# SelennLamson/AntsRL

Hardware: AMD Instinct MI355X
Metric: ant-steps/sec (ants x envs x steps/s), 256^2 grid (higher is better)
Workload: dtype f64 ant kinematics / f32 grids

## Files before the change

antsrl_amd/csrc/antsrl_capi.hip:

```cpp
#include <hip/hip_runtime.h>
#include <stdarg.h>
#include <stdio.h>
#include <math.h>
#include <stdlib.h>
#include <string.h>
#include <new>

#include "antsrl_device.h"

hipError_t antsrl_launch_act(const KP &p, const int8_t *rot, const int8_t *ph, int cur, float *obs,
                             float *agent_state, float *reward, uint8_t *done, int flags,
                             const double *jitter, int out_buf, hipStream_t st);
bool antsrl_act_fits(const KP &p);
bool antsrl_act_needs_hbm_maps(const KP &p);
hipError_t antsrl_launch_sweep(const KP &p, int cur, hipStream_t st);
hipError_t antsrl_launch_update(const KP &p, const double *jitter, int out_buf, hipStream_t st, int phases = 15);
hipError_t antsrl_launch_collect_full(const KP &p, hipStream_t st);
hipError_t antsrl_launch_reset(const KP &p, const AntsInit *in, hipStream_t st);
hipError_t antsrl_launch_set_activation(const KP &p, const float *act, hipStream_t st);
hipError_t antsrl_launch_read_state(const KP &p, int which, int cur, void *dst, hipStream_t st);
hipError_t antsrl_launch_perceptive_field(const KP &p, uint8_t *dst, hipStream_t st);
hipError_t antsrl_launch_generate(const KP &p, const AntsGen &g, uint64_t seed, hipStream_t st);
hipError_t antsrl_launch_phero_wall_clear(const KP &p, hipStream_t st, int buf = 0);
hipError_t antsrl_launch_phero_renorm(const KP &p, hipStream_t st);
bool antsrl_meta_supported(const KP &p);
hipError_t antsrl_launch_move(const KP &p, const int8_t *rot, const int8_t *ph, uint8_t *done, int do_step, uint32_t seq,
                              hipStream_t st);
hipError_t antsrl_launch_perceive(const KP &p, int cur, float *obs, float *agent_state, float *reward, int flags,
                                  uint32_t seq, hipStream_t st, const PolArgs *pol, uint32_t obs_pitch);
bool antsrl_inloop_policy_supported(const KP &p);
hipError_t antsrl_launch_policy_pack(unsigned char *pack, const float *w1, const float *b1, const float *w2, const float *b2,
                                     const float *w3, const float *b3, int F, hipStream_t st);
hipError_t antsrl_launch_meta_rebase(const KP &p, hipStream_t st);
bool antsrl_update_move_supported(const KP &p);
hipError_t antsrl_launch_update_move(const KP &p, int out_buf, double g_dep, double inv_g_dep, const int8_t *rot,
                                     const int8_t *ph, uint8_t *done, uint32_t seq, hipStream_t st, bool with_frames);
int antsrl_perceive_run(const KP &p);
hipError_t antsrl_launch_copy16(void *dst, const void *src, size_t bytes, hipStream_t st);

struct AntsHandle {
    AntsCfg cfg;
    KP p;
    int cur;
    int steps_since_update;
    bool need_full_collect;
    bool is_reset;
    bool episode_over;
    size_t ws_bytes;
    AntsGen gen;
    bool has_gen;
    uint64_t episode_seed;
    int host_timestep;
    long long sweeps;
    bool obs_bf16;
    uint32_t obs_pitch;
    bool need_wall_clear;
    hipEvent_t ev[ANTSRL_TIMING_EVENTS];
    bool ev_armed;
    uint32_t obs_seq;
    PolArgs pol;
    bool pend_update;
    KP pend_p;
    int pend_out_buf;
    int phase_next;
};

static thread_local char g_err[512] = "";

static int fail(int code, const char *fmt, ...)
{
    va_list ap;
    va_start(ap, fmt);
    vsnprintf(g_err, sizeof(g_err), fmt, ap);
    va_end(ap);
    return code;
}

static int hip_fail(hipError_t e, const char *what)
{
    return fail(ANTSRL_E_DEVICE, "%s: %s", what, hipGetErrorString(e));
}

extern "C" int antsrl_abi_version(void) { return ANTSRL_ABI_VERSION; }
extern "C" size_t antsrl_cfg_size(void) { return sizeof(AntsCfg); }
extern "C" const char *antsrl_last_error(void) { return g_err; }

static void fill_kp(const AntsCfg *c, KP *p);

static int validate(const AntsCfg *c)
{
    if (!c) return fail(ANTSRL_E_INVALID, "cfg is NULL");
    if (c->abi_version != ANTSRL_ABI_VERSION)
        return fail(ANTSRL_E_INVALID, "AntsCfg.abi_version %d != library %d", c->abi_version, ANTSRL_ABI_VERSION);
    if (c->n_envs < 1 || c->n_ants < 1 || c->w < 1 || c->h < 1)
        return fail(ANTSRL_E_INVALID, "n_envs, n_ants, w, h must be >= 1");
    if ((long long)c->w * c->h > (1ll << 30)) return fail(ANTSRL_E_INVALID, "grid too large");
    if (c->n_envs > 65535)
        return fail(ANTSRL_E_INVALID, "n_envs must be <= 65535 per handle (shard larger batches over handles / GPUs)");
    if (c->n_phero < 1 || c->n_phero > ANTSRL_MAX_PHERO)
        return fail(ANTSRL_E_INVALID, "n_phero must be in 1..%d", ANTSRL_MAX_PHERO);
    if (c->n_rocks < 0 || c->n_rocks > 32) return fail(ANTSRL_E_INVALID, "n_rocks must be in 0..32");
    if (c->perception_radius < 0 || 2 * c->perception_radius + 1 > ANTSRL_MAX_PSIDE)
        return fail(ANTSRL_E_INVALID, "perception side must be <= %d", ANTSRL_MAX_PSIDE);
    if (c->n_channels < 1 || c->n_channels > ANTSRL_MAX_CHANNELS)
        return fail(ANTSRL_E_INVALID, "n_channels must be in 1..%d", ANTSRL_MAX_CHANNELS);
    for (int k = 0; k < c->n_channels; ++k) {
        const int kind = c->channel_kind[k];
        if (kind < ANTSRL_CH_ANTS || kind > ANTSRL_CH_ROCKS) return fail(ANTSRL_E_INVALID, "bad channel kind");
        if (kind == ANTSRL_CH_PHERO && (c->channel_arg[k] < 0 || c->channel_arg[k] >= c->n_phero))
            return fail(ANTSRL_E_INVALID, "pheromone channel index out of range");
        if (kind == ANTSRL_CH_PHERO && !c->has_max_val)
            return fail(ANTSRL_E_INVALID, "a perceived pheromone needs max_val (RL_api.py:125 divides by it)");
        if (kind == ANTSRL_CH_ROCKS && c->n_rocks == 0)
            return fail(ANTSRL_E_INVALID, "rocks perceived but n_rocks == 0");
    }
    if (c->filter_radius < 0 || c->filter_radius > ANTSRL_MAX_FILTER_RADIUS)
        return fail(ANTSRL_E_INVALID, "filter_radius must be in 0..%d", ANTSRL_MAX_FILTER_RADIUS);
    if (c->reward_kind < ANTSRL_REWARD_NONE || c->reward_kind > ANTSRL_REWARD_ALL)
        return fail(ANTSRL_E_INVALID, "bad reward_kind");
    if (c->has_max_val && !(c->phero_max_val > 0)) return fail(ANTSRL_E_INVALID, "phero_max_val must be > 0");
    if (c->act_path < ANTSRL_ACT_AUTO || c->act_path > ANTSRL_ACT_SINGLE_KERNEL) return fail(ANTSRL_E_INVALID, "bad act_path");
    if (c->env_id_base < 0 || (long long)c->env_id_base + c->n_envs > 0x7fffffffll)
        return fail(ANTSRL_E_INVALID, "env_id_base must be >= 0 and env_id_base + n_envs must fit 31 bits");
    if (c->n_envs_total != 0 && (long long)c->n_envs_total < (long long)c->env_id_base + c->n_envs)
        return fail(ANTSRL_E_INVALID, "n_envs_total %d < env_id_base + n_envs = %lld (0 = that sum)", c->n_envs_total,
                    (long long)c->env_id_base + c->n_envs);
    if (c->act_path == ANTSRL_ACT_CELL_META) {
        KP kp;
        fill_kp(c, &kp);
        if (!kp.meta)
            return fail(ANTSRL_E_UNSUPPORTED, "ANTSRL_ACT_CELL_META needs 2 pheromone channels, the generator's channel order "
                                              "([Ants, Phero0, Phero1, Anthill, Walls, Food(, Rocks)]), a perception of 128..368 values "
                                              "per ant over at most 64 cells, and at most 4096 ants per env");
    }
    return ANTSRL_OK;
}

static bool use_scaled(const AntsCfg *c)
{
    return c->phero_mode == ANTSRL_PHERO_AUTO && c->filter_radius == 0 && c->filter[0] > 0.5 &&
           c->filter[0] <= 1.0 && c->phero_threshold >= 0.0;
}

static bool use_interleaved(const AntsCfg *c)
{
    static const bool off = PROF_ENV("ANTSRL_NO_INTERLEAVE") != nullptr;
    return !off && use_scaled(c) && c->n_phero == 2;
}

static size_t carve(const AntsCfg *c, DState *s, unsigned char *base)
{
    const size_t E = c->n_envs, N = c->n_ants, G = (size_t)c->w * c->h, Cn = c->n_phero, R = c->n_rocks;
    const size_t words = (G + 31) / 32;
    size_t off = 0;
    auto take = [&](size_t bytes) -> unsigned char * {
        unsigned char *ptr = base ? base + off : nullptr;
        off = (off + bytes + 255) / 256 * 256;
        return ptr;
    };
// ... 190 lines not shown
{
    if (!h || !init) return fail(ANTSRL_E_INVALID, "NULL handle or init");
    if (!init->ants_xyt || !init->seed || !init->walls || !init->food || !init->anthill_xyr)
        return fail(ANTSRL_E_INVALID, "AntsInit: ants_xyt, seed, walls, food, anthill_xyr are required");
    if (h->p.R > 0 && !init->rocks) return fail(ANTSRL_E_INVALID, "AntsInit.rocks is NULL but n_rocks > 0");
    h->pend_update = false;
    h->phase_next = 0;
    hipError_t e = antsrl_launch_reset(h->p, init, (hipStream_t)stream);
    if (e != hipSuccess) return hip_fail(e, "reset");
    h->p.deposit_strength = h->cfg.deposit_strength;
    h->cur = 0; h->steps_since_update = 0; h->need_full_collect = true; h->is_reset = true; h->episode_over = false;
    h->sweeps = 0; h->need_wall_clear = h->p.scaled && init->phero != nullptr;
    h->host_timestep = 1; h->obs_seq = 0;
    set_decay(h);
    return ANTSRL_OK;
}

static int check_gen_seed(const AntsHandle *h, const AntsGen &g, uint64_t seed)
{
    const uint64_t top = (uint64_t)h->p.env_id_base + (uint64_t)h->p.E;
    const uint64_t lim = 0xFFFFFFFFull / 5u;
    if (g.rng_kind == ANTSRL_RNG_REFERENCE && (top > lim || seed > lim - top))
        return fail(ANTSRL_E_INVALID, "ANTSRL_RNG_REFERENCE: (episode_seed + env_id_base + n_envs) * 5 must stay below 2^32 (np.random.seed)");
    return ANTSRL_OK;
}

static int do_generate(AntsHandle *h, uint64_t seed, hipStream_t st)
{
    int rc = check_gen_seed(h, h->gen, seed);
    if (rc) return rc;
    h->pend_update = false;
    h->phase_next = 0;
    hipError_t e = antsrl_launch_generate(h->p, h->gen, seed, st);
    if (e != hipSuccess) return hip_fail(e, "generate");
    h->p.deposit_strength = h->cfg.deposit_strength;
    h->cur = 0; h->steps_since_update = 0; h->need_full_collect = true; h->is_reset = true; h->episode_over = false;
    h->sweeps = 0; h->need_wall_clear = false; h->host_timestep = 1; h->obs_seq = 0;
    h->episode_seed = seed;
    set_decay(h);
    return ANTSRL_OK;
}

extern "C" int antsrl_generate(AntsHandle *h, const AntsGen *gen, uint64_t episode_seed, void *stream)
{
    if (!h || !gen) return fail(ANTSRL_E_INVALID, "NULL handle or gen");
    if (gen->n_food_discs < 0 || gen->n_food_discs > ANTSRL_MAX_FOOD_DISCS)
        return fail(ANTSRL_E_INVALID, "n_food_discs must be in 0..%d", ANTSRL_MAX_FOOD_DISCS);
    if (gen->food_rmin < 0 || gen->food_rmax < gen->food_rmin) return fail(ANTSRL_E_INVALID, "bad food radii");
    if (gen->wall_kind == ANTSRL_WALLS_BERNOULLI) {
        if (!(gen->wall_density >= 0.0 && gen->wall_density <= 1.0)) return fail(ANTSRL_E_INVALID, "bad wall_density");
    } else if (gen->wall_kind == ANTSRL_WALLS_PERLIN) {
        if (!(gen->wall_density >= -1.0 && gen->wall_density <= 1.0) || gen->perlin_octaves < 1 || gen->perlin_octaves > 8 ||
            !(gen->perlin_scale > 0.0) || !(gen->perlin_persistence > 0.0) || !(gen->perlin_lacunarity > 0.0))
            return fail(ANTSRL_E_INVALID, "bad Perlin wall parameters (density in [-1, 1], 1..8 octaves, positive "
                                          "scale / persistence / lacunarity)");
    } else if (gen->wall_kind == ANTSRL_WALLS_INPUT) {
        if (!gen->walls_input) return fail(ANTSRL_E_INVALID, "ANTSRL_WALLS_INPUT needs AntsGen.walls_input");
    } else {
        return fail(ANTSRL_E_INVALID, "bad wall_kind %d", gen->wall_kind);
    }
    if (gen->rng_kind != ANTSRL_RNG_COUNTER && gen->rng_kind != ANTSRL_RNG_REFERENCE)
        return fail(ANTSRL_E_INVALID, "bad rng_kind %d", gen->rng_kind);
    if (gen->rng_kind == ANTSRL_RNG_REFERENCE) {
        if (gen->wall_kind == ANTSRL_WALLS_BERNOULLI && gen->wall_density != 0.0)
            return fail(ANTSRL_E_UNSUPPORTED, "the reference has no Bernoulli walls generator: with ANTSRL_RNG_REFERENCE use "
                                              "ANTSRL_WALLS_PERLIN, ANTSRL_WALLS_INPUT or wall_density 0");
    }
    int rc = check_gen_seed(h, *gen, episode_seed);
    if (rc) return rc;
    h->gen = *gen;
    h->has_gen = true;
    return do_generate(h, episode_seed, (hipStream_t)stream);
}

static int bf16_unsupported()
{
    return fail(ANTSRL_E_UNSUPPORTED, "bfloat16 observations on the single-kernel path (k_act) need 2 pheromone channels, the "
                                      "generator's channel order ([Ants, Phero0, Phero1, Anthill, Walls, Food(, Rocks)]), a perception of "
                                      "at most 64 cells and a grid whose bit maps fit LDS (up to ~600k cells); the cell-meta path "
                                      "(ANTSRL_Q_CELL_META) has no grid limit");
}

extern "C" int antsrl_set_obs_format(AntsHandle *h, int format)
{
    if (!h) return fail(ANTSRL_E_INVALID, "NULL handle");
    if (format != ANTSRL_OBS_F32 && format != ANTSRL_OBS_BF16) return fail(ANTSRL_E_INVALID, "bad observation format %d", format);
    if ((format == ANTSRL_OBS_BF16) != h->obs_bf16) h->obs_pitch = 0;
    h->obs_bf16 = format == ANTSRL_OBS_BF16;
    if (!h->obs_bf16) h->pol = PolArgs{};
    return ANTSRL_OK;
}

extern "C" int antsrl_set_obs_row_stride(AntsHandle *h, int32_t stride_elems)
{
    if (!h) return fail(ANTSRL_E_INVALID, "NULL handle");
    const int32_t row = h->p.PP * h->p.K, esz = h->obs_bf16 ? 2 : 4;
    if (stride_elems == 0 || stride_elems == row) {
        h->obs_pitch = 0;
        return ANTSRL_OK;
    }
    if (stride_elems < row || ((long long)stride_elems * esz) % 128 != 0 || stride_elems > row + 128 / esz)
        return fail(ANTSRL_E_INVALID, "obs row stride %d: 0 (dense) or the row's %d elements rounded up to whole 128-byte lines (%d)",
                    stride_elems, row, (row * esz + 127) / 128 * 128 / esz);
    if (!h->p.meta) return fail(ANTSRL_E_UNSUPPORTED, "antsrl_set_obs_row_stride needs the cell-meta path (ANTSRL_Q_CELL_META)");
    if (h->pol.pack)
        return fail(ANTSRL_E_UNSUPPORTED, "a padded observation row stride and the in-loop policy exclude each other (the net reads a "
                                          "dense tile image): switch the policy off first (antsrl_set_inloop_policy with w1 == NULL)");
    h->obs_pitch = (uint32_t)stride_elems;
    return ANTSRL_OK;
}

static int hip_fail(hipError_t e, const char *what);
static int flush_pending(AntsHandle *h, hipStream_t st)
{
    if (!h->pend_update) return ANTSRL_OK;
    h->pend_update = false;
    hipError_t e = antsrl_launch_update(h->pend_p, nullptr, h->pend_out_buf, st);
    if (e != hipSuccess) return hip_fail(e, "deferred update");
    return ANTSRL_OK;
}

static int not_reset(const AntsHandle *h)
{
    if (h->episode_over)
        return fail(ANTSRL_E_INVALID, "the episode is over and its auto-reset was refused (episode seed past np.random.seed's 32 bits): "
                                      "call antsrl_reset or antsrl_generate");
    return fail(ANTSRL_E_INVALID, "antsrl_reset has not been called on this handle");
}

static int mid_update(const AntsHandle *h)
{
    return fail(ANTSRL_E_INVALID, "an Environment.update is in progress (antsrl_update_phase %d of 4 is next): finish it first", h->phase_next);
}

static int meta_observe(AntsHandle *h, const int8_t *rot, const int8_t *ph, float *obs, float *agent_state,
                        float *reward, uint8_t *done, bool stepping, hipStream_t st, bool timed)
{
    hipError_t e;
    if (obs && h->obs_pitch != 0 && h->obs_pitch != (uint32_t)(h->p.PP * h->p.K) && h->pol.pack && h->obs_bf16)
        return fail(ANTSRL_E_UNSUPPORTED, "a padded observation row stride and the in-loop policy exclude each other");
    if (h->obs_seq >= META_NEVER - 2) {
        e = antsrl_launch_meta_rebase(h->p, st);
        if (e != hipSuccess) return hip_fail(e, "explored-stamp rebase");
        h->obs_seq = 0;
    }
    h->obs_seq++;
    bool frames = false;
    if (h->pend_update && stepping) {
        h->pend_update = false;
        frames = h->pol.pack != nullptr;
        if (const char *s = PROF_ENV("ANTSRL_FRAMES")) frames = atoi(s) != 0;
        e = antsrl_launch_update_move(h->p, h->pend_out_buf, h->pend_p.g_dep, h->pend_p.inv_g_dep, rot, ph, done, h->obs_seq, st, frames);
        if (e != hipSuccess) return hip_fail(e, "update + move");
    } else {
        int rc = flush_pending(h, st);
        if (rc) return rc;
        e = antsrl_launch_move(h->p, rot, ph, done, stepping ? 1 : 0, h->obs_seq, st);
        if (e != hipSuccess) return hip_fail(e, "move");
    }
    if (timed) (void)hipEventRecord(h->ev[2], st);
    e = antsrl_launch_perceive(h->p, h->cur, obs, agent_state, reward,
                               (stepping ? ACT_STEP : 0) | (obs ? ACT_HAS_OBS : 0) | (frames ? ACT_FRAMES : 0) |
                                   ((obs || h->pol.pack) && h->obs_bf16 ? ACT_OBS_BF16 : 0),
                               h->obs_seq, st, &h->pol, h->obs_pitch);
    if (e == hipErrorNotSupported)
        return fail(ANTSRL_E_UNSUPPORTED, "a padded observation row stride and the in-loop policy exclude each other (the net reads a dense tile image)");
    if (e != hipSuccess) return hip_fail(e, "perceive");
    return ANTSRL_OK;
}

static int do_step(AntsHandle *h, const int8_t *rot, const int8_t *ph, float *obs, float *agent_state,
                   float *reward, uint8_t *done, hipStream_t st, bool fused_update = false,
                   const double *jitter = nullptr, bool timed = false)
{
    if (ph && h->p.C != 2)
        return fail(ANTSRL_E_INVALID, "pheromone actions need exactly 2 pheromone channels (ants.py:89-96)");
    if (h->steps_since_update > 0) h->need_full_collect = true;
    if (h->p.meta) {
        int rc = meta_observe(h, rot, ph, obs, agent_state, reward, done, true, st, timed);
        if (rc) return rc;
        h->steps_since_update++;
        return ANTSRL_OK;
    }
    if (obs && h->obs_pitch) return fail(ANTSRL_E_UNSUPPORTED, "antsrl_set_obs_row_stride needs the cell-meta path (ANTSRL_Q_CELL_META)");
    if (timed) (void)hipEventRecord(h->ev[2], st);
    static const int ablate = PROF_ENV("ANTSRL_ABLATE") ? atoi(PROF_ENV("ANTSRL_ABLATE")) & ~15 : 0;
    hipError_t e = antsrl_launch_act(h->p, rot, ph, h->cur, obs, agent_state, reward, done,
                                     ACT_STEP | (obs ? ACT_HAS_OBS : 0) | (fused_update ? ACT_FUSED_UPDATE : 0) | ablate |
                                         (obs && h->obs_bf16 ? ACT_OBS_BF16 : 0),
                                     jitter, h->p.scaled ? 0 : h->cur ^ 1, st);
    if (e == hipErrorNotSupported) return bf16_unsupported();
    if (e != hipSuccess) return hip_fail(e, "step");
    h->steps_since_update++;
    return ANTSRL_OK;
}

static int do_update(AntsHandle *h, const double *jitter, hipStream_t st, bool sweep_done,
                     bool update_fused = false, bool may_defer = false)
{
    hipError_t e;
    int frc = flush_pending(h, st);
    if (frc) return frc;
    if (h->p.scaled) {
        if (h->p.g_dep < 1e-20) {
            e = antsrl_launch_phero_renorm(h->p, st);
            if (e != hipSuccess) return hip_fail(e, "pheromone renorm");
            h->sweeps = 0;
            set_decay(h);
        }
        if (h->need_wall_clear) {
            e = antsrl_launch_phero_wall_clear(h->p, st);
            if (e != hipSuccess) return hip_fail(e, "pheromone wall clear");
            h->need_wall_clear = false;
        }
    } else if (!sweep_done) {
        e = antsrl_launch_sweep(h->p, h->cur, st);
        if (e != hipSuccess) return hip_fail(e, "pheromone sweep");
    }
    if (!update_fused) {
        if (may_defer && !jitter && !h->need_full_collect && antsrl_update_move_supported(h->p)) {
            h->pend_update = true;
            h->pend_p = h->p;
            h->pend_out_buf = h->p.scaled ? 0 : h->cur ^ 1;
        } else {
            e = antsrl_launch_update(h->p, jitter, h->p.scaled ? 0 : h->cur ^ 1, st);
            if (e != hipSuccess) return hip_fail(e, "update");
        }
    }
    if (h->p.scaled) {
        h->sweeps++;
        set_decay(h);
    }
    if (h->need_full_collect) {
        e = antsrl_launch_collect_full(h->p, st);
        if (e != hipSuccess) return hip_fail(e, "anthill collect");
        h->need_full_collect = false;
    }
    if (!h->p.scaled) h->cur ^= 1;
    h->steps_since_update = 0;
    h->host_timestep++;
    return ANTSRL_OK;
}

extern "C" int antsrl_step(AntsHandle *h, const int8_t *rotation, const int8_t *phero, float *obs,
                           float *agent_state, float *reward, uint8_t *done, void *stream)
{
    if (!h) return fail(ANTSRL_E_INVALID, "NULL handle");
    if (!h->is_reset) return not_reset(h);
    if (h->phase_next) return mid_update(h);
    if (!agent_state || !reward || !done) return fail(ANTSRL_E_INVALID, "agent_state, reward, done are required");
    return do_step(h, rotation, phero, obs, agent_state, reward, done, (hipStream_t)stream);
}

extern "C" int antsrl_observe(AntsHandle *h, float *obs, float *agent_state, float *reward, void *stream)
{
    if (!h) return fail(ANTSRL_E_INVALID, "NULL handle");
    if (!h->is_reset) return not_reset(h);
    if (h->phase_next) return mid_update(h);
    if (h->p.meta)
        return meta_observe(h, nullptr, nullptr, obs, agent_state, reward, nullptr, false, (hipStream_t)stream, false);
    if (obs && h->obs_pitch) return fail(ANTSRL_E_UNSUPPORTED, "antsrl_set_obs_row_stride needs the cell-meta path (ANTSRL_Q_CELL_META)");
    hipError_t e = antsrl_launch_act(h->p, nullptr, nullptr, h->cur, obs, agent_state, reward, nullptr,
                                     obs ? ACT_HAS_OBS | (h->obs_bf16 ? ACT_OBS_BF16 : 0) : 0, nullptr, 0,
                                     (hipStream_t)stream);
    if (e == hipErrorNotSupported) return bf16_unsupported();
    if (e != hipSuccess) return hip_fail(e, "observe");
    return ANTSRL_OK;
}

extern "C" int antsrl_update(AntsHandle *h, const double *wall_jitter, void *stream)
{
    if (!h) return fail(ANTSRL_E_INVALID, "NULL handle");
    if (!h->is_reset) return not_reset(h);
    if (h->phase_next) return mid_update(h);
    return do_update(h, wall_jitter, (hipStream_t)stream, false, false, true);
}

extern "C" int antsrl_update_phase(AntsHandle *h, int phase, const double *wall_jitter, void *stream)
{
    if (!h) return fail(ANTSRL_E_INVALID, "NULL handle");
    if (!h->is_reset) return not_reset(h);
    if (phase < ANTSRL_PHASE_WALLS || phase > ANTSRL_PHASE_ANTHILL) return fail(ANTSRL_E_INVALID, "bad phase %d", phase);
    if (phase != h->phase_next)
        return fail(ANTSRL_E_INVALID, "antsrl_update_phase: phase %d is next, got %d (WALLS, ROCKS_PHEROMONE, ANTS, ANTHILL in order)", h->phase_next, phase);
    hipStream_t st = (hipStream_t)stream;
    hipError_t e;
    if (phase == ANTSRL_PHASE_WALLS) {
        int frc = flush_pending(h, st);
        if (frc) return frc;
        if (h->p.scaled) {
            if (h->p.g_dep < 1e-20) {
                e = antsrl_launch_phero_renorm(h->p, st);
                if (e != hipSuccess) return hip_fail(e, "pheromone renorm");
                h->sweeps = 0;
                set_decay(h);
            }
            if (h->need_wall_clear) {
                e = antsrl_launch_phero_wall_clear(h->p, st);
                if (e != hipSuccess) return hip_fail(e, "pheromone wall clear");
                h->need_wall_clear = false;
            }
        } else {
            e = antsrl_launch_phero_wall_clear(h->p, st, h->cur);
            if (e != hipSuccess) return hip_fail(e, "pheromone wall clear");
        }
        e = antsrl_launch_update(h->p, wall_jitter, h->p.scaled ? 0 : h->cur, st, 1 );
// ... 240 lines not shown
```

antsrl_amd/csrc/antsrl_perceive.hip:

```cpp
#include "antsrl_util.h"
#include "antsrl_flush.h"
#include "antsrl_update_one.h"

#define PRC_UNROLL 2

constexpr bool abl_gather = (PRC_ABL & 1) != 0, abl_store = (PRC_ABL & 2) != 0, abl_mark = (PRC_ABL & 4) != 0;

#define PLAYOUT_DEFAULT 1
#define PLAYOUT_DEFAULT_ROCKS 2

__host__ __device__ inline size_t move_lds_bytes(int HT, int N)
{
    return align_up(8 * (size_t)HT + 12 * (size_t)N, 16);
}

template <int C>
__device__ __forceinline__ void move_body(const KP &p, const int e, const int8_t *__restrict__ rotation,
                                          const int8_t *__restrict__ phero_act, uint8_t *__restrict__ done, const int do_step,
                                          const uint32_t seq, unsigned char *smem, const UmFwd *fw = nullptr)
{
    const int tid = threadIdx.x, T = blockDim.x;
    const int N = p.N, W = p.W, H = p.H;
    const size_t G = (size_t)W * H, eN = (size_t)e * N;
    uint32_t *hkeys = (uint32_t *)smem, *hvals = hkeys + p.HT;
    float *tmp_q = (float *)(hvals + p.HT), *tmp_d = tmp_q + N;
    uint32_t *cprevs = (uint32_t *)(tmp_d + N);

    const uint32_t *area = p.s.area_bits + (size_t)e * p.words;
    const FoodView food{p.s.food + (size_t)e * G * p.fs, p.fs};
    uint16_t *pres = reinterpret_cast<uint16_t *>(p.s.food + (size_t)e * G * p.fs) + 2;
    const size_t FS2 = 2 * (size_t)p.fs;

    const bool one = fw ? true : N <= T;
    const size_t a1 = eN + (tid < N ? tid : 0);
    double h_x = 0.0, h_y = 0.0, h_th = 0.0;
    float h_hold = 0.0f, h_q = 0.0f;
    int h_m = 0, h_rot = 0, h_pa = 0;
    uint32_t h_cprev = 0u;
    if (one) {
        if (fw) {
            h_x = fw->x; h_y = fw->y; h_th = fw->th;
            h_hold = fw->hold; h_m = fw->m & 1; h_rot = fw->rot; h_pa = fw->pa;
            h_cprev = frec_xy(p, (int)fw->x, (int)fw->y);
            if (fw->rec) h_q = (UM_ABL & 1) ? 0.0f : ((fw->meta & META_AREA) ? 0.0f : fw->food);
            else h_q = (UM_ABL & 1) ? 0.0f : food[h_cprev];
        } else {
            h_x = p.s.x[a1]; h_y = p.s.y[a1]; h_th = p.s.theta[a1];
            h_hold = p.s.holding[a1];
            if (do_step) {
                const double ppx = STP_LD(p.s.prev_x[a1]), ppy = STP_LD(p.s.prev_y[a1]);
                h_m = STP_LD(p.s.mandibles[a1]);
                if (rotation) h_rot = STP_LD(rotation[a1]);
                if (phero_act) h_pa = STP_LD(phero_act[a1]);
                h_cprev = frec_xy(p, (int)ppx, (int)ppy);
                h_q = (UM_ABL & 1) ? 0.0f : food[h_cprev];
            }
        }
    }
    if (do_step && !fw)
        for (int h = tid; h < p.HT; h += T) {
            hkeys[h] = HASH_EMPTY;
            hvals[h] = 0u;
        }
    if (tid == 0) {
        if (p.reward_kind != ANTSRL_REWARD_NONE) {
            p.s.primed_cur[e] = fw ? fw->primed : p.s.reward_primed[e];
            p.s.reward_primed[e] = 1;
        }
        if (do_step && done) done[e] = (uint8_t)(p.max_time == (fw ? fw->ts : p.s.timestep[e]));
    }
    if (!fw) __syncthreads();
    else __builtin_amdgcn_sched_barrier(0);
    if (fw) UM_STAMP(10);

    if (do_step) {
        for (int i = tid; i < N; i += T) {
            double x, y;
            uint32_t cprev;
            float q, hold;
            int old_m;
            if (one) {
                x = h_x; y = h_y; cprev = h_cprev; q = h_q; old_m = h_m; hold = h_hold;
            } else {
                x = p.s.x[eN + i]; y = p.s.y[eN + i];
                cprev = frec_xy(p, (int)p.s.prev_x[eN + i], (int)p.s.prev_y[eN + i]);
                q = food[cprev];
                old_m = p.s.mandibles[eN + i];
                hold = p.s.holding[eN + i];
            }
            const uint32_t ccur = (uint32_t)((int)x * H + (int)y);
            int m = old_m;
            {
                const int set = q > 0.0f;
                const int keep = 1 - (int)((fw && fw->rec) ? (fw->meta & META_AREA) != 0 : test_bit(area, ccur));
                if (p.mand_first == 1) m |= set;
                else if (p.mand_first == 2) m &= keep;
                if (p.mand_last == 1) m |= set;
                else if (p.mand_last == 2) m &= keep;
            }
            const int closing = m & (1 - old_m), opening = (1 - m) & old_m;
            const float taken = fminf((float)p.max_hold, fmaxf(0.0f, q)) * (float)closing;
            const float dropped = hold * (float)opening;
            h_hold = hold + (taken - dropped);
            p.s.holding[eN + i] = h_hold;
            STP_ST(p.s.mandibles[eN + i], (uint8_t)m);
            cprevs[i] = cprev;
            tmp_q[i] = q;
            tmp_d[i] = dropped - taken;
            if (fw) break;
            lww_insert(hkeys, hvals, (uint32_t)p.HT - 1, cprev, (uint32_t)i);
        }
        if (!fw) __syncthreads();
        else __builtin_amdgcn_sched_barrier(0);
        if (fw) UM_STAMP(11);
        for (int i = tid; i < N; i += T) {
            const uint32_t cprev = cprevs[i];
            const float delta = tmp_d[i];
            int32_t dirty = -1;
            if (delta != 0.0f && (fw ? (fw->m & UMFWD_WIN) != 0 : lww_winner(hkeys, hvals, (uint32_t)p.HT - 1, cprev) == (uint32_t)i)) {
                food[cprev] = tmp_q[i] + delta;
                if (__float_as_uint((&food[cprev])[1]) & META_AREA) dirty = (int32_t)cprev;
            }
            STP_ST(p.s.dirty_cell[eN + i], dirty);
            if (fw) break;
        }
        if (fw) UM_STAMP(12);
    }

    for (int i = tid; i < N; i += T) {
        double x, y, th;
        if (one) {
            x = h_x; y = h_y; th = h_th;
        } else {
            x = p.s.x[eN + i]; y = p.s.y[eN + i]; th = p.s.theta[eN + i];
        }
        if (do_step) {
            if (phero_act) {
                const int a = one ? h_pa : (int)phero_act[eN + i];
                float a0 = 0.0f, a1 = 0.0f;
                if (a == 1) a0 = (float)p.deposit_strength;
                else if (a != 0) a1 = (float)p.deposit_strength;
                STP_ST(p.s.activation[(eN + i) * C + 0], a0);
                if (C > 1) STP_ST(p.s.activation[(eN + i) * C + 1], a1);
            }
            double sn, cs;
            if (fw && fw->pre) {
                th = fw->th_new; sn = fw->sn; cs = fw->cs;
            } else {
                if (rotation)
                    th = np_mod_d(th + (double)(one ? h_rot : (int)rotation[eN + i]) * p.max_rot_speed, 2 * PI_D);
                sincos(th, &sn, &cs);
            }
            double fwd = 1.0 * p.max_speed * (1 - (double)(one ? h_hold : p.s.holding[eN + i]) * p.carry);
            if (fwd < 0) fwd *= p.backward;
            x = warp_coord(x + cs * fwd, (double)W);
            y = warp_coord(y + sn * fwd, (double)H);
            p.s.x[eN + i] = x;
            p.s.y[eN + i] = y;
            p.s.theta[eN + i] = th;
        }
        const uint32_t cell = frec_xy(p, wrap_index((int)x, W), wrap_index((int)y, H));
        if (!(UM_ABL & 2) || cell == 0xFFFFFFFFu) pres[(size_t)cell * FS2] = (uint16_t)seq;
        if (fw && fw->frm_off) {
            const double *fs = reinterpret_cast<const double *>(smem + fw->frm_off) + 2 * i;
            AntFrame f;
            const bool shifted = p.fwd_delta != 0.0;
            f.cx = shifted ? x + fw->cs * p.fwd_delta : x;
            f.cy = shifted ? y + fw->sn * p.fwd_delta : y;
            f.ct = fs[0];
            f.st = fs[1];
            p.s.frames[eN + i] = f;
        }
        if (fw) break;
    }
    if (fw) UM_STAMP(13);
}

template <int C>
__global__ void __launch_bounds__(1024)
k_move(const KP p, const int8_t *__restrict__ rotation, const int8_t *__restrict__ phero_act,
       uint8_t *__restrict__ done, const int do_step, const uint32_t seq)
{
    extern __shared__ __align__(16) unsigned char smem[];
    move_body<C>(p, env_of_block(blockIdx.x, p.E, seq), rotation, phero_act, done, do_step, seq, smem);
}

template <int C, bool ILV>
__global__ void __launch_bounds__(1024, 8)
k_update_move(const KP p, const int out_buf, const double g_dep, const double inv_g_dep, const int8_t *__restrict__ rotation,
              const int8_t *__restrict__ phero_act, uint8_t *__restrict__ done, const uint32_t seq, const int with_frames)
{
    extern __shared__ __align__(16) unsigned char smem[];
    const int e = env_of_block(blockIdx.x, p.E, seq);
    UM_STAMP(0);
    UmFwd fw = {};
    {
        const size_t a = (size_t)e * p.N + (threadIdx.x < (unsigned)p.N ? threadIdx.x : 0);
        fw.hold = p.s.holding[a];
        fw.m = STP_LD(p.s.mandibles[a]);
        if (rotation) fw.rot = STP_LD(rotation[a]);
        if (phero_act) fw.pa = STP_LD(phero_act[a]);
        fw.has_rot = rotation != nullptr;
        fw.primed = p.s.reward_primed[e];
    }
    fw.rec = (ILV && C == 2 && !(UM_ABL & 4)) ? 1 : 0;
    fw.frm_off = with_frames ? (uint32_t)align_up(max(update_one_lds_bytes(p.HT, p.R, (int)(blockDim.x >> 6), p.N), move_lds_bytes(p.HT, p.N)), 16) : 0u;
    update_one_body<C, ILV>(p, e, nullptr, out_buf, smem, g_dep, inv_g_dep, &fw);
    __syncthreads();
    UM_STAMP(9);
    move_body<C>(p, e, rotation, phero_act, done, 1, seq, smem, &fw);
#ifdef UM_TRACE
    __builtin_amdgcn_s_waitcnt(0x0F70);
    UM_STAMP(14);
    if (threadIdx.x == 0 && blockIdx.x < UM_TRACE_MAX_WGS) g_um_trace[blockIdx.x * UM_TRACE_SLOTS + 15] = __builtin_amdgcn_s_getreg(4 | (31 << 11));
#endif
}

struct PrcOff {
    uint32_t rock, wave0, frame, rm, stage, per_wave, stride;
    size_t total;
};

__host__ __device__ __forceinline__ PrcOff prc_offsets(int run, int PP, int K, int R, int nwaves, bool no_stage = false, uint32_t pitch = 0)
{
    PrcOff o;
    o.rock = 0;
    o.wave0 = (uint32_t)(32 * (size_t)(R > 0 ? R : 1));
    o.frame = 0;
    o.rm = (uint32_t)(sizeof(AntFrame) * (size_t)run);
    o.stage = (uint32_t)align_up(o.rm + (R > 0 ? 4 * (size_t)run : 0), 16);
    const size_t rowf = (size_t)PP * K;
    o.stride = (uint32_t)((2 * rowf + 32 + 3) / 4 * 4);
    if (2 * pitch > o.stride) o.stride = 2 * pitch;
    o.per_wave = (uint32_t)align_up(o.stage + (no_stage ? 0 : 4 * (size_t)o.stride), 16);
    o.total = o.wave0 + (size_t)nwaves * o.per_wave;
    return o;
}

__host__ __device__ __forceinline__ uint32_t prc_policy_img_elems(int row) { return (uint32_t)((32 * row + 8 + 32 + 7) / 8 * 8); }

#define PRC_TPB 256

__device__ __forceinline__ int prc_tile_ant(const int w, const int j, const int run, const int nwaves)
{
    (void)nwaves;
    return w * run + j;
}

typedef __attribute__((ext_vector_type(8))) __bf16 prc_bf16x8;
typedef __attribute__((ext_vector_type(16))) float prc_f32x16;
typedef __attribute__((ext_vector_type(4))) uint32_t prc_u4;

__device__ __forceinline__ void policy_tile(const PolArgs &pol, const uint16_t *img, const uint32_t img_shift, const float *as_lds,
                                            const int F, const int rows, const size_t ant0, const int lane)
{
    const int r = lane & 31, h = lane >> 5;
    const prc_u4 *wpack = reinterpret_cast<const prc_u4 *>(pol.pack);
    const prc_u4 *a2pack = reinterpret_cast<const prc_u4 *>(pol.pack + ANTSRL_POL_WPACK_BYTES);
    const float *lanepack = reinterpret_cast<const float *>(pol.pack + ANTSRL_POL_WPACK_BYTES + ANTSRL_POL_A2PACK_BYTES);
    const int rc = min(r, rows - 1);
    const float as0 = (float)(__bf16)as_lds[2 * rc], as1 = (float)(__bf16)as_lds[2 * rc + 1];
    prc_f32x16 acc;
#pragma unroll
    for (int g = 0; g < 16; ++g) acc[g] = 0.0f;
    const uint32_t off0 = img_shift + (uint32_t)r * (uint32_t)F + 8u * h;
    const int ks = pol.ks;
    constexpr int POL_AHEAD = 6;
    prc_u4 a[POL_AHEAD];
#pragma unroll
    for (int i = 0; i < POL_AHEAD; ++i) a[i] = wpack[min(i, ks - 1) * 64 + lane];
    for (int s0 = 0; s0 < ks; s0 += POL_AHEAD) {
#pragma unroll
        for (int i = 0; i < POL_AHEAD; ++i) {
            const int s = s0 + i;
            const prc_u4 a_s = a[i];
            a[i] = wpack[min(s + POL_AHEAD, ks - 1) * 64 + lane];
            if (s < ks) {
                const uint32_t off = off0 + 16u * s, sh = (off & 1u) * 16u;
                const uint32_t *d = reinterpret_cast<const uint32_t *>(img) + (off >> 1);
                const uint32_t d0 = d[0], d1 = d[1], d2 = d[2], d3 = d[3], d4 = d[4];
                const prc_u4 packed = {__builtin_amdgcn_alignbit(d1, d0, sh), __builtin_amdgcn_alignbit(d2, d1, sh),
                                       __builtin_amdgcn_alignbit(d3, d2, sh), __builtin_amdgcn_alignbit(d4, d3, sh)};
                acc = __builtin_amdgcn_mfma_f32_32x32x16_bf16(__builtin_bit_cast(prc_bf16x8, a_s),
                                                              __builtin_bit_cast(prc_bf16x8, packed), acc, 0, 0, 0);
            }
        }
    }
    prc_f32x16 acc2;
#pragma unroll
    for (int g = 0; g < 16; ++g) acc2[g] = 0.0f;
#pragma unroll
    for (int s = 0; s < 2; ++s) {
        prc_bf16x8 hfrag;
#pragma unroll
        for (int j = 0; j < 8; ++j) {
            const int g = 8 * s + j;
            const float bias1 = lanepack[g * 64 + lane], was0 = lanepack[(16 + g) * 64 + lane], was1 = lanepack[(32 + g) * 64 + lane];
            hfrag[j] = (__bf16)(acc[g] + (as0 * was0 + as1 * was1) + bias1);
        }
        acc2 = __builtin_amdgcn_mfma_f32_32x32x16_bf16(__builtin_bit_cast(prc_bf16x8, a2pack[s * 64 + lane]), hfrag, acc2, 0, 0, 0);
    }
    float lg[6];
    lg[0] = acc2[0]; lg[1] = acc2[1]; lg[2] = acc2[2]; lg[3] = acc2[3];
    lg[4] = __shfl(acc2[0], r + 32); lg[5] = __shfl(acc2[1], r + 32);
#pragma unroll
    for (int o = 0; o < 6; ++o) lg[o] += lanepack[48 * 64 + o];
    if (h == 0 && r < rows) {
        int ar = 0, ap = 0;
        if (lg[1] > lg[ar]) ar = 1;
        if (lg[2] > lg[ar]) ar = 2;
        if (lg[4] > lg[3 + ap]) ap = 1;
// ... 635 lines not shown
```

antsrl_amd/csrc/antsrl_update_one.h:

```cpp
#pragma once
#include "antsrl_util.h"
#include "antsrl_update_env.h"

__host__ __device__ inline size_t update_one_lds_bytes(int HT, int R, int nwaves, int N)
{
    return align_up(8 * (size_t)HT, 16) + 48 * (size_t)(R > 0 ? R : 1) + 8 * (size_t)nwaves +
           align_up(4 * (size_t)nwaves, 8) + 16 * (size_t)N + align_up(4 * (size_t)R, 16) + 16;
}

template <int C, bool FWD_REC = false>
__device__ __forceinline__ void update_one_body(const KP &p, const int e, const double *__restrict__ wall_jitter, const int out_buf,
                                                unsigned char *smem, const double g_dep, const double inv_g_dep, UmFwd *fw = nullptr)
{
    const int tid = threadIdx.x, T = blockDim.x;
    const int lane = tid & 63, wave = __builtin_amdgcn_readfirstlane(tid >> 6), nwaves = T >> 6;
    const int N = p.N, W = p.W, H = p.H, R = p.R;
    const size_t G = (size_t)W * H, eN = (size_t)e * N;
    uint32_t *hkeys = (uint32_t *)smem, *hvals = hkeys + p.HT;
    double *rock = (double *)(smem + align_up(8 * (size_t)p.HT, 16));
    double *rk = rock + 4 * (R > 0 ? R : 1);
    double *red = rk + 2 * (R > 0 ? R : 1);
    uint32_t *wave_tot = (uint32_t *)(red + nwaves);
    double *sx = (double *)((unsigned char *)wave_tot + align_up(4 * (size_t)nwaves, 8)), *sy = sx + N;
    uint32_t *rk_hit = (uint32_t *)(sy + N);

    const uint32_t *walls = p.s.walls_bits + (size_t)e * p.words;
    const FoodView food{p.s.food + (size_t)e * G * p.fs, p.fs};
    const size_t PS = (size_t)p.ps;
    float *out = p.s.phero[out_buf] + (size_t)e * G * PS;
    const bool on = tid < N;
    const size_t a = eN + (on ? tid : 0);

    double x = p.s.x[a], y = p.s.y[a];
    const double px0 = STP_LD(p.s.prev_x[a]), py0 = STP_LD(p.s.prev_y[a]);
    const uint8_t rstate = STP_LD(p.s.reward_state[a]);
    const double theta0 = p.s.theta[a];
    float act[C];
#pragma unroll
    for (int c = 0; c < C; ++c) act[c] = STP_LD(p.s.activation[a * C + c]);
    const int32_t wc_l = STP_LD(p.s.walldep_cell[a]), dc_l = STP_LD(p.s.dirty_cell[a]);
    const int32_t wc = (p.scaled && on) ? wc_l : -1;
    const int32_t dc = on ? dc_l : -1;
    const int ts = p.s.timestep[e] + 1;
    if (tid < R) {
        rock[4 * tid + 0] = p.s.rock_cx[(size_t)e * R + tid];
        rock[4 * tid + 1] = p.s.rock_cy[(size_t)e * R + tid];
        rock[4 * tid + 2] = p.s.rock_r[(size_t)e * R + tid];
        rock[4 * tid + 3] = p.s.rock_w[(size_t)e * R + tid];
    }
    for (int h = tid; h < p.HT; h += T) {
        hkeys[h] = HASH_EMPTY;
        hvals[h] = 0u;
    }
    const float food_dc_l = food[dc_l >= 0 ? dc_l : 0];
    const float food_dc = dc >= 0 ? food_dc_l : 0.0f;

    const bool hit = on && test_bit(walls, (uint32_t)((int)x * H + (int)y));
    UM_STAMP(1);
    double u = 0.0;
    if (wall_jitter) {
        uint32_t tot;
        const uint32_t rank = block_excl_scan_flag(hit, wave_tot, lane, wave, nwaves, &tot);
        if (hit) u = wall_jitter[eN + rank];
    } else if (hit) {
        u = jitter_u01(p.rng_seed, p.env_id_base + (uint32_t)e, (uint32_t)ts, (uint32_t)tid);
    }
    bool moved = hit;
    if (hit) {
        x = px0;
        y = py0;
        if (!fw) p.s.theta[a] = theta0 + (u - 0.5);
    }
    if (fw) fw->th = hit ? theta0 + (u - 0.5) : theta0;
    UM_STAMP_ON(2, (int)hit);

    if (R > 0) {
        if (on) {
            sx[tid] = x;
            sy[tid] = y;
        }
        __syncthreads();
        UM_STAMP(3);
        for (int q = wave; q < R; q += nwaves) {
            const double cx = rock[4 * q + 0], cy = rock[4 * q + 1], rad = rock[4 * q + 2];
            const double rad2_hi = rad * rad * (1.0 + 1e-12) + 1e-300;
            double sumx = 0.0, sumy = 0.0;
            bool any = false;
            for (int base = 0; base < N; base += 64) {
                const int i = base + lane;
                double px = 0.0, py = 0.0;
                bool col = false;
                if (i < N) {
                    const double vx = cx - sx[i], vy = cy - sy[i];
                    const double d2 = vx * vx + vy * vy;
                    if (!(d2 > rad2_hi)) {
                        const double d = sqrt(d2);
                        const double f = 1 - rad / (d + 0.001);
                        px = vx * f; py = vy * f;
                        col = !(d > rad);
                    }
                }
                unsigned long long m = __ballot(col);
                any |= m != 0;
                while (m) {
                    const int l = __builtin_ctzll(m);
                    m &= m - 1;
                    sumx += __shfl(px, l);
                    sumy += __shfl(py, l);
                }
            }
            if (lane == 0) {
                rk[2 * q + 0] = cx - sumx / rock[4 * q + 3];
                rk[2 * q + 1] = cy - sumy / rock[4 * q + 3];
                rk_hit[q] = any ? 1u : 0u;
            }
        }
        __syncthreads();
        UM_STAMP(4);
        if (tid < R) {
            p.s.rock_cx[(size_t)e * R + tid] = rk[2 * tid + 0];
            p.s.rock_cy[(size_t)e * R + tid] = rk[2 * tid + 1];
        }
        double ax = 0.0, ay = 0.0;
        for (int q = 0; q < R; ++q) {
            if (!rk_hit[q]) continue;
            const double vx = rk[2 * q + 0] - x, vy = rk[2 * q + 1] - y;
            const double rad = rock[4 * q + 2];
            const double d2 = vx * vx + vy * vy;
            if (d2 > rad * rad * (1.0 + 1e-12) + 1e-300) continue;
            const double d = sqrt(d2);
            const double f = 1 - rad / (d + 0.001);
            double px = vx * f, py = vy * f;
            if (d > rad) { px = 0.0; py = 0.0; }
            ax += px; ay += py;
        }
        x = warp_coord(x + ax, (double)W);
        y = warp_coord(y + ay, (double)H);
        moved = true;
        UM_STAMP(5);
    }

    __syncthreads();
    const uint32_t cell_id = (uint32_t)((int)x * H + (int)y);
    const uint32_t cell = prec_xy(p, (int)x, (int)y);
    float pold[C];
    constexpr bool fw_rec = FWD_REC && C == 2 && !(UM_ABL & 4);
    if constexpr (fw_rec) {
        const stream_f4 rec = *reinterpret_cast<const stream_f4 *>(out + (size_t)cell * 4);
        pold[0] = rec.x;
        pold[C - 1] = rec.y;
        fw->food = rec.z;
        fw->meta = __float_as_uint(rec.w);
    } else {
#pragma unroll
        for (int c = 0; c < C; ++c) pold[c] = (UM_ABL & 4) ? 0.0f : out[(size_t)cell * PS + c];
    }
    if (fw) {
        double th = fw->th;
        if (fw->has_rot) th = np_mod_d(th + (double)fw->rot * p.max_rot_speed, 2 * PI_D);
        fw->th_new = th;
        sincos(th, &fw->sn, &fw->cs);
        fw->pre = 1;
        fw->ts = ts;
        if (fw->frm_off) {
            double st2, ct2;
            sincos(th + PI_D * 0.5, &st2, &ct2);
            double *fs = reinterpret_cast<double *>(smem + fw->frm_off) + 2 * tid;
            fs[0] = ct2;
            fs[1] = st2;
        }
    }
    if (on) {
        if (moved && !fw) {
            p.s.x[a] = x;
            p.s.y[a] = y;
        }
        STP_ST(p.s.prev_x[a], x);
        STP_ST(p.s.prev_y[a], y);
        if (fw) {
            fw->x = x;
            fw->y = y;
        }
        lww_insert(hkeys, hvals, (uint32_t)p.HT - 1, cell, (uint32_t)tid);
        STP_ST(p.s.reward_state[a], (uint8_t)((double)rstate * 0.9));
    }
    __syncthreads();
    UM_STAMP(6);
    if (p.scaled) {
        if (wc >= 0) {
            for (int c = 0; c < C; ++c) out[(size_t)wc * PS + c] = 0.0f;
            p.s.walldep_cell[a] = -1;
        }
        __syncthreads();
        UM_STAMP(7);
    }
    if constexpr (fw_rec) {
        asm volatile("" : "+v"(pold[0]), "+v"(pold[C - 1]), "+v"(fw->food), "+v"(fw->meta));
    }
    double gain = 0.0;
    if (on) {
        const bool winner = lww_winner(hkeys, hvals, (uint32_t)p.HT - 1, cell) == (uint32_t)tid;
        if (fw && winner) fw->m |= UMFWD_WIN;
        if (winner) {
            if (!p.scaled) {
#pragma unroll
                for (int c = 0; c < C; ++c) {
                    if (act[c] != 0.0f) {
                        float v = pold[c] + act[c];
                        if (p.has_max_val) v = fminf(v, (float)p.max_val);
                        out[(size_t)cell * PS + c] = v;
                    }
                }
            } else {
                bool on_wall;
                if constexpr (fw_rec) on_wall = (fw->meta & META_WALL) != 0;
                else on_wall = test_bit(walls, cell_id);
                bool wrote = false;
#pragma unroll
                for (int c = 0; c < C; ++c) {
                    if (act[c] != 0.0f) {
                        double v = (double)pold[c] * g_dep;
                        if (v < p.threshold || on_wall) v = 0.0;
                        v += (double)act[c];
                        if (p.has_max_val) v = fmin(v, p.max_val);
                        if (!(UM_ABL & 4) || v == 12345.678) out[(size_t)cell * PS + c] = (float)(v * inv_g_dep);
                        wrote = true;
                    } else if (on_wall) {
                        out[(size_t)cell * PS + c] = 0.0f;
                    }
                }
                if (on_wall && wrote) p.s.walldep_cell[a] = (int32_t)cell;
            }
        }
        if (dc >= 0) {
            gain = (double)food_dc;
            food[dc] = 0.0f;
            p.s.dirty_cell[a] = -1;
        }
    }
    UM_STAMP(8);
    for (int o = 32; o > 0; o >>= 1) gain += __shfl_down(gain, o);
    if (lane == 0) red[wave] = gain;
    __syncthreads();
    if (tid == 0) {
        double s2 = 0.0;
        for (int w = 0; w < nwaves; ++w) s2 += red[w];
        if (s2 != 0.0) p.s.anthill_food[e] += s2;
        p.s.timestep[e] = ts;
    }
}
```

Before: 2.682 billion.

## Ping-pong x/prev_x buffers and skip unchanged state stores in fused update-move

The fused update+move path no longer writes both x and prev_x every step. Post-update positions stay in the x array and are stored only when they actually changed, while the move step writes the new positions into prev_x, and the host swaps the two pointers after launch. Stores of holding, mandibles, dirty_cell and reward_state are also skipped when the value is unchanged, and a __syncthreads is restored for the non-record fused case. This cuts HBM write traffic per ant step, but it adds data-dependent branches and depends on the pointer swap staying consistent with every other reader of x and prev_x.

```diff
diff --git a/antsrl_amd/csrc/antsrl_capi.hip b/antsrl_amd/csrc/antsrl_capi.hip
--- a/antsrl_amd/csrc/antsrl_capi.hip
+++ b/antsrl_amd/csrc/antsrl_capi.hip
@@ -5,6 +5,7 @@
 #include <stdlib.h>
 #include <string.h>
 #include <new>
+#include <utility>
 
 #include "antsrl_device.h"
 
@@ -501,6 +502,8 @@
         if (const char *s = PROF_ENV("ANTSRL_FRAMES")) frames = atoi(s) != 0;
         e = antsrl_launch_update_move(h->p, h->pend_out_buf, h->pend_p.g_dep, h->pend_p.inv_g_dep, rot, ph, done, h->obs_seq, st, frames);
         if (e != hipSuccess) return hip_fail(e, "update + move");
+        std::swap(h->p.s.x, h->p.s.prev_x);
+        std::swap(h->p.s.y, h->p.s.prev_y);
     } else {
         int rc = flush_pending(h, st);
         if (rc) return rc;
diff --git a/antsrl_amd/csrc/antsrl_perceive.hip b/antsrl_amd/csrc/antsrl_perceive.hip
--- a/antsrl_amd/csrc/antsrl_perceive.hip
+++ b/antsrl_amd/csrc/antsrl_perceive.hip
@@ -102,15 +102,15 @@
             const float taken = fminf((float)p.max_hold, fmaxf(0.0f, q)) * (float)closing;
             const float dropped = hold * (float)opening;
             h_hold = hold + (taken - dropped);
-            p.s.holding[eN + i] = h_hold;
-            STP_ST(p.s.mandibles[eN + i], (uint8_t)m);
+            if (__float_as_uint(h_hold) != __float_as_uint(hold)) p.s.holding[eN + i] = h_hold;
+            if (m != old_m) STP_ST(p.s.mandibles[eN + i], (uint8_t)m);
             cprevs[i] = cprev;
             tmp_q[i] = q;
             tmp_d[i] = dropped - taken;
             if (fw) break;
             lww_insert(hkeys, hvals, (uint32_t)p.HT - 1, cprev, (uint32_t)i);
         }
-        if (!fw) __syncthreads();
+        if (!fw || !fw->rec) __syncthreads();
         else __builtin_amdgcn_sched_barrier(0);
         if (fw) UM_STAMP(11);
         for (int i = tid; i < N; i += T) {
@@ -121,7 +121,7 @@
                 food[cprev] = tmp_q[i] + delta;
                 if (__float_as_uint((&food[cprev])[1]) & META_AREA) dirty = (int32_t)cprev;
             }
-            STP_ST(p.s.dirty_cell[eN + i], dirty);
+            if (!fw || dirty >= 0) STP_ST(p.s.dirty_cell[eN + i], dirty);
             if (fw) break;
         }
         if (fw) UM_STAMP(12);
@@ -155,8 +155,8 @@
             if (fwd < 0) fwd *= p.backward;
             x = warp_coord(x + cs * fwd, (double)W);
             y = warp_coord(y + sn * fwd, (double)H);
-            p.s.x[eN + i] = x;
-            p.s.y[eN + i] = y;
+            (fw ? p.s.prev_x : p.s.x)[eN + i] = x;
+            (fw ? p.s.prev_y : p.s.y)[eN + i] = y;
             p.s.theta[eN + i] = th;
         }
         const uint32_t cell = frec_xy(p, wrap_index((int)x, W), wrap_index((int)y, H));
diff --git a/antsrl_amd/csrc/antsrl_update_one.h b/antsrl_amd/csrc/antsrl_update_one.h
--- a/antsrl_amd/csrc/antsrl_update_one.h
+++ b/antsrl_amd/csrc/antsrl_update_one.h
@@ -66,6 +66,7 @@
         u = jitter_u01(p.rng_seed, p.env_id_base + (uint32_t)e, (uint32_t)ts, (uint32_t)tid);
     }
     bool moved = hit;
+    bool chg = hit && (__double_as_longlong(px0) != __double_as_longlong(x) || __double_as_longlong(py0) != __double_as_longlong(y));
     if (hit) {
         x = px0;
         y = py0;
@@ -134,8 +135,10 @@
             if (d > rad) { px = 0.0; py = 0.0; }
             ax += px; ay += py;
         }
-        x = warp_coord(x + ax, (double)W);
-        y = warp_coord(y + ay, (double)H);
+        const double wx = warp_coord(x + ax, (double)W), wy = warp_coord(y + ay, (double)H);
+        chg = chg || __double_as_longlong(wx) != __double_as_longlong(x) || __double_as_longlong(wy) != __double_as_longlong(y);
+        x = wx;
+        y = wy;
         moved = true;
         UM_STAMP(5);
     }
@@ -171,18 +174,24 @@
         }
     }
     if (on) {
-        if (moved && !fw) {
-            p.s.x[a] = x;
-            p.s.y[a] = y;
-        }
-        STP_ST(p.s.prev_x[a], x);
-        STP_ST(p.s.prev_y[a], y);
-        if (fw) {
+        if (!fw) {
+            if (moved) {
+                p.s.x[a] = x;
+                p.s.y[a] = y;
+            }
+            STP_ST(p.s.prev_x[a], x);
+            STP_ST(p.s.prev_y[a], y);
+        } else {
+            if (chg) {
+                p.s.x[a] = x;
+                p.s.y[a] = y;
+            }
             fw->x = x;
             fw->y = y;
         }
         lww_insert(hkeys, hvals, (uint32_t)p.HT - 1, cell, (uint32_t)tid);
-        STP_ST(p.s.reward_state[a], (uint8_t)((double)rstate * 0.9));
+        const uint8_t rs = (uint8_t)((double)rstate * 0.9);
+        if (rs != rstate) STP_ST(p.s.reward_state[a], rs);
     }
     __syncthreads();
     UM_STAMP(6);
```

New measurement: 2.682 billion (median of 4 runs). Within noise of the previous version (+0.0%).
